# chrismile/LineVis

Hardware: AMD Instinct MI355X
Metric: Mrays/s (higher is better)
Workload: dtype f32

## Files before the change

### linevis_amd/csrc/lv_api.hip

```cpp
#include <algorithm>
#include <cmath>
#include <cstdlib>
#include <cstring>

#include "lv_internal.h"
#include "lv_trace.h"
#include "lv_mboit.h"

int lv_fail(lv_ctx* ctx, int code, const char* fmt, ...) {
    char buf[1024];
    va_list ap;
    va_start(ap, fmt);
    vsnprintf(buf, sizeof(buf), fmt, ap);
    va_end(ap);
    if (ctx) ctx->lastError = buf;
    return code;
}

int lv_buf_reserve(lv_ctx* ctx, LvDeviceBuffer& b, size_t bytes) {
    if (bytes == 0) bytes = 16;
    if (b.ptr && b.bytes >= bytes) return LV_OK;
    if (b.ptr) {
        LV_HIP(ctx, hipStreamSynchronize(ctx->stream));
        (void)hipFree(b.ptr);
// ... 33 lines not shown
    float c14 = m[4] * m[15] - m[12] * m[7];
    float c15 = m[4] * m[11] - m[8] * m[7];
    float c16 = m[8] * m[14] - m[12] * m[10];
    float c18 = m[4] * m[14] - m[12] * m[6];
    float c19 = m[4] * m[10] - m[8] * m[6];
    float c20 = m[8] * m[13] - m[12] * m[9];
    float c22 = m[4] * m[13] - m[12] * m[5];
    float c23 = m[4] * m[9] - m[8] * m[5];

    float i00 = +((m[5] * c00 - m[6] * c04) + m[7] * c08);
    float i01 = -((m[1] * c00 - m[2] * c04) + m[3] * c08);
    float i02 = +((m[1] * c02 - m[2] * c06) + m[3] * c10);
    float i03 = -((m[1] * c03 - m[2] * c07) + m[3] * c11);
    float i10 = -((m[4] * c00 - m[6] * c12) + m[7] * c16);
    float i11 = +((m[0] * c00 - m[2] * c12) + m[3] * c16);
    float i12 = -((m[0] * c02 - m[2] * c14) + m[3] * c18);
    float i13 = +((m[0] * c03 - m[2] * c15) + m[3] * c19);
    float i20 = +((m[4] * c04 - m[5] * c12) + m[7] * c20);
    float i21 = -((m[0] * c04 - m[1] * c12) + m[3] * c20);
    float i22 = +((m[0] * c06 - m[1] * c14) + m[3] * c22);
    float i23 = -((m[0] * c07 - m[1] * c15) + m[3] * c23);
    float i30 = -((m[4] * c08 - m[5] * c16) + m[6] * c20);
    float i31 = +((m[0] * c08 - m[1] * c16) + m[2] * c20);
    float i32 = -((m[0] * c10 - m[1] * c18) + m[2] * c22);
    float i33 = +((m[0] * c11 - m[1] * c19) + m[2] * c23);

    float det = ((m[0] * i00 + m[1] * i10) + m[2] * i20) + m[3] * i30;
    float r = 1.0f / det;
    inv[0] = i00 * r;  inv[1] = i01 * r;  inv[2] = i02 * r;  inv[3] = i03 * r;
    inv[4] = i10 * r;  inv[5] = i11 * r;  inv[6] = i12 * r;  inv[7] = i13 * r;
    inv[8] = i20 * r;  inv[9] = i21 * r;  inv[10] = i22 * r; inv[11] = i23 * r;
    inv[12] = i30 * r; inv[13] = i31 * r; inv[14] = i32 * r; inv[15] = i33 * r;
    return det;
}

static bool lv_mat4_invertible(const float* m, const float* inv, float det) {
    float hadamard = 1.0f;
    for (int c = 0; c < 4; c++) hadamard *= sqrtf(((m[4 * c] * m[4 * c] + m[4 * c + 1] * m[4 * c + 1]) + m[4 * c + 2] * m[4 * c + 2]) + m[4 * c + 3] * m[4 * c + 3]);
    for (int i = 0; i < 16; i++)
        if (!std::isfinite(m[i]) || !std::isfinite(inv[i])) return false;
    return std::isfinite(det) && std::isfinite(hadamard) && fabsf(det) > 1e-5f * hadamard;
}

static std::vector<LvDeviceBuffer*> lv_all_buffers(lv_ctx* ctx) {
    return {&ctx->points, &ctx->segIdx, &ctx->nodes, &ctx->segs, &ctx->segAxis, &ctx->prismFrames, &ctx->leafSeg, &ctx->segToLeaf, &ctx->tf,
            &ctx->depthMinMax, &ctx->ao, &ctx->aoAlt, &ctx->featNormal, &ctx->featNormalAlt, &ctx->featPosition, &ctx->featPositionAlt,
            &ctx->eawPing, &ctx->eawPong, &ctx->tilesHaloDev, &ctx->fullFrameTile, &ctx->svgf.normalDepth, &ctx->svgf.normalDepthHistory,
            &ctx->svgf.flowFwidth, &ctx->svgf.moments, &ctx->svgf.momentsHistory, &ctx->svgf.colorHistory, &ctx->svgf.tempAccum,
            &ctx->svgf.tempAccumFiltered, &ctx->svgf.ping, &ctx->svgf.pong, &ctx->svgf.result, &ctx->svgfGiven, &ctx->aoGbuf, &ctx->aoList, &ctx->aoSamples,
            &ctx->counters, &ctx->ppllNodes, &ctx->ppllStart, &ctx->ppllCount, &ctx->ppllScratch, &ctx->prismRecords, &ctx->scanTemp, &ctx->ppllOverflow, &ctx->mlabLong, &ctx->mlabStatsSnap, &ctx->mboitAccum, &ctx->ppllCoarse, &ctx->prismLeafList, &ctx->flowOccupancy, &ctx->flowPoints, &ctx->flowPointsNext, &ctx->flowSelfGrid, &ctx->twistTex, &ctx->tilesDev, &ctx->outDev,
            &ctx->scratchRays, &ctx->stackOverflow, &ctx->trajPos, &ctx->trajAttr, &ctx->trajOff, &ctx->trajLineValid, &ctx->trajLineRef, &ctx->trajRecLine, &ctx->trajTess, &ctx->trajRibbon, &ctx->trajHelicity, &ctx->trajMaxHelicity, &ctx->trajRecPoint, &ctx->trajMeshRot, &ctx->triIdx, &ctx->triVerts, &ctx->triPoints, &ctx->triNodes, &ctx->tris, &ctx->triPairFlag,
            &ctx->flowVectors, &ctx->flowScalars, &ctx->flowMisc, &ctx->flowSeeds, &ctx->flowOutPos, &ctx->flowOutAtt, &ctx->flowCounts,
            &ctx->bakeBlendingWeights, &ctx->bakeSamplingLocations, &ctx->bakedAo, &ctx->bakeLcgSkip, &ctx->bakedAoPending, &ctx->bakeCounters,
            &ctx->bakeGbuf, &ctx->bakeSamples, &ctx->bakeOverflow, &ctx->mlatTrace, &ctx->buildArena, &ctx->firstHit,
            &ctx->accum, &ctx->selftestIn, &ctx->selftestOut, &ctx->groupOrder[0].cost, &ctx->groupOrder[0].order, &ctx->groupOrder[1].cost, &ctx->groupOrder[1].order};
}

namespace {

typedef LvDevCounters LvDevCountersHost;

bool parseBool(const char* v) { return strcmp(v, "true") == 0 || strcmp(v, "1") == 0; }

bool parseFloat(const char* v, float& out) {
    char* end = nullptr;
    float f = strtof(v, &end);
    if (end == v) return false;
    out = f;
    return true;
}
bool parseUint(const char* v, uint32_t& out) {
    char* end = nullptr;
    long long x = strtoll(v, &end, 10);
    if (end == v || x < 0 || x > 0xFFFFFFFFll) return false;
    out = uint32_t(x);
    return true;
}

void updateAoMode(lv_ctx* ctx) {
    ctx->opt.useAmbientOcclusion = ctx->opt.aoBakerIsRtao && ctx->opt.aoStrength > 0.0f;
}

}

extern "C" {

const char* lv_version(void) { return "linevis_hip 0.1 (gfx950)"; }

lv_ctx* lv_create(int device_ordinal, int* err) {
    int n = 0;
    hipError_t e = hipGetDeviceCount(&n);
    if (e != hipSuccess || n <= 0 || device_ordinal < 0 || device_ordinal >= n) {
        if (err) *err = LV_E_HIP;
        return nullptr;
    }
    if (hipSetDevice(device_ordinal) != hipSuccess) {
        if (err) *err = LV_E_HIP;
        return nullptr;
    }
    lv_ctx* ctx = new lv_ctx();
    ctx->device = device_ordinal;
    {
        hipDeviceProp_t prop;
        if (hipGetDeviceProperties(&prop, device_ordinal) == hipSuccess && prop.multiProcessorCount > 0)
            ctx->numCUs = prop.multiProcessorCount;
    }
    memset(&ctx->stats, 0, sizeof(ctx->stats));
// ... 563 lines not shown
        if (p != o.triLeafPairs) { ctx->triAccelValid = false; lv_invalidate_bake(ctx); }
        o.triLeafPairs = p;
    } else if (k == "treelet_leaves") {
        uint32_t t;
        if (!parseUint(value, t) || t < 3 || t > 4096) return bad();
        if (t != o.treeletLeaves) { ctx->accelValid = false; ctx->triAccelValid = false; lv_invalidate_bake(ctx); }
        o.treeletLeaves = t;
    } else if (k == "treelet_lane_leaves") {
        uint32_t t;
        if (!parseUint(value, t) || t == 1 || t > 64) return bad();
        if (t != o.treeletLaneLeaves) { ctx->accelValid = false; ctx->triAccelValid = false; lv_invalidate_bake(ctx); }
        o.treeletLaneLeaves = t;
    } else if (k == "treelet_group_leaves") {
        uint32_t t;
        if (!parseUint(value, t) || (t != 0 && t != 8 && t != 16)) return bad();
        if (t != o.treeletGroupLeaves) { ctx->accelValid = false; ctx->triAccelValid = false; lv_invalidate_bake(ctx); }
        o.treeletGroupLeaves = t;
    } else if (k == "kernel_timers") {
        const std::string v(value);
        uint32_t mask = 0u;
        if (v == "all") mask = 0xFFFFFFFFu;
        else if (v != "none") {
            size_t pos = 0;
            while (pos <= v.size()) {
                size_t e = v.find(',', pos);
                if (e == std::string::npos) e = v.size();
                const std::string t = v.substr(pos, e - pos);
                pos = e + 1;
                uint32_t id;
                if (t == "phases") mask |= 1u << 31;
                else if (parseUint(t.c_str(), id) && id < 31u) mask |= 1u << id;
                else return bad();
            }
        }
        o.timerMask = mask;
    } else if (k == "accel_collapse_top") {
        const bool b = parseBool(value);
        if (b != o.collapseTop) { ctx->accelValid = false; ctx->triAccelValid = false; lv_invalidate_bake(ctx); }
        o.collapseTop = b;
    } else if (k == "treelet_plane_eval") {
        bool sc;
        if (std::string(value) == "scan") sc = true;
        else if (std::string(value) == "loop") sc = false;
        else return bad();
        if (sc != o.treeletPlaneScan) { ctx->accelValid = false; ctx->triAccelValid = false; lv_invalidate_bake(ctx); }
        o.treeletPlaneScan = sc;
    } else if (k == "accel_build") {
        bool ft;
        if (std::string(value) == "fast_trace") ft = true;
        else if (std::string(value) == "fast_build") ft = false;
        else return bad();
        if (ft != o.accelFastTrace) { ctx->accelValid = false; ctx->triAccelValid = false; lv_invalidate_bake(ctx); }
        o.accelFastTrace = ft;
    } else if (k == "dispatch_order") {
        if (std::string(value) == "cost") o.dispatchByCost = true;
        else if (std::string(value) == "as_numbered") o.dispatchByCost = false;
        else return bad();
    } else if (k == "rtao_geometry") {
        if (std::string(value) == "auto") o.rtaoGeometry = 0;
        else if (std::string(value) == "capsules") o.rtaoGeometry = 1;
        else if (std::string(value) == "triangle_tubes") o.rtaoGeometry = 2;
        else return bad();
    } else {
        return lv_fail(ctx, LV_E_INVALID, "unknown option '%s'", key);
    }
    return lv_forward_to_ranks(ctx, [&](lv_ctx* p) { return lv_set_option(p, key, value); });
}

int lv_build_accel(lv_ctx* ctx) {
    if (!ctx) return LV_E_INVALID;
    (void)hipSetDevice(ctx->device);
    int rc = lv_ensure_line_points(ctx);
    if (rc) return rc;
    if ((rc = lv_bvh_build(ctx))) return rc;
    const bool needTriangles = (ctx->opt.useAmbientOcclusion && (ctx->opt.aoPrebaked || lv_ao_triangle_tubes(ctx))) || ctx->opt.rtTriangleMesh;
    if (needTriangles) {
        if ((rc = lv_ensure_tube_mesh(ctx))) return rc;
        if (ctx->triMeshSet && (rc = lv_bvh_build_triangles(ctx))) return rc;
    }
    return lv_forward_to_ranks(ctx, [&](lv_ctx* p) { return lv_build_accel(p); });
}

lv_ctx* lv_create_multi(const int* device_ordinals, int num_devices, const char* transport, int* err) {
    if (!device_ordinals || num_devices <= 0) {
        if (err) *err = LV_E_INVALID;
        return nullptr;
    }
    lv_ctx* ctx = lv_create(device_ordinals[0], err);
    if (!ctx) return nullptr;
    const int rc = lv_multi_create(ctx, device_ordinals, num_devices, transport);
    if (rc) {
        fprintf(stderr, "lv_create_multi: %s\n", ctx->lastError.c_str());
        lv_destroy(ctx);
        if (err) *err = rc;
        return nullptr;
    }
    if (err) *err = LV_OK;
    return ctx;
}

int lv_multi_ranks(const lv_ctx* ctx) { return ctx ? lv_multi_num_ranks(ctx) : 0; }

int lv_multi_rebalance(lv_ctx* ctx, double base_cost_per_tile) {
    if (!ctx) return LV_E_INVALID;
    return lv_multi_rebalance_impl(ctx, base_cost_per_tile);
}
// ... 606 lines not shown
```

### linevis_amd/csrc/lv_bvh.hip

```cpp
#include <algorithm>
#include <cstring>
#include <utility>

#include <rocprim/device/device_radix_sort.hpp>
#include <rocprim/device/device_scan.hpp>

#include "lv_internal.h"

namespace {

__device__ __forceinline__ void lv_block_bounds(const float mn[3], const float mx[3], uint32_t* boundsOrd) {
    __shared__ float s_red[6][LV_BLOCK / LV_WAVE];
#pragma unroll
    for (int k = 0; k < 3; k++) {
        const float a = lv_wave_min(mn[k]), b = lv_wave_max(mx[k]);
        if (lv_lane() == 0) { s_red[k][threadIdx.x >> 6] = a; s_red[3 + k][threadIdx.x >> 6] = b; }
    }
    __syncthreads();
    if (threadIdx.x < 6) {
        float v = s_red[threadIdx.x][0];
        for (int w = 1; w < LV_BLOCK / LV_WAVE; w++)
            v = threadIdx.x < 3 ? fminf(v, s_red[threadIdx.x][w]) : fmaxf(v, s_red[threadIdx.x][w]);
        if (threadIdx.x < 3) atomicMin(&boundsOrd[threadIdx.x], lv_f2ord(v));
        else atomicMax(&boundsOrd[threadIdx.x], lv_f2ord(v));
// ... 774 lines not shown
                    const bool valid = j < hi;
                    bool left = false;
                    uint32_t e = 0;
                    if (valid) {
                        e = s_idx[j];
                        const float* b = s_box[e];
                        const int bi = int(((b[ax] + b[3 + ax]) - cmn[ax]) * scale[ax]);
                        const uint32_t bn = uint32_t(bi < 0 ? 0 : (bi > int(LV_TREELET_BINS) - 1 ? int(LV_TREELET_BINS) - 1 : bi));
                        left = bn < plane;
                    }
                    const unsigned long long mL = __ballot(left), mR = __ballot(valid && !left);
                    if (valid) {
                        if (left) s_tmp[lo + runL + uint32_t(__popcll(mL & below))] = e;
                        else s_tmp[lo + nl + runR + uint32_t(__popcll(mR & below))] = e;
                    }
                    runL += uint32_t(__popcll(mL));
                    runR += uint32_t(__popcll(mR));
                }
                LV_TREELET_SYNC();
                for (uint32_t j = lo + lane; j < hi; j += 64u) s_idx[j] = s_tmp[j];
                LV_TREELET_SYNC();
                if (nl == 0u || nl == n) nl = n / 2u;
            }
        }
        const uint32_t nr = n - nl;
        const uint32_t sL = nl > 1u ? v++ : 0u, sR = nr > 1u ? v++ : 0u;
        if (lane == 0u) {
            childL[slot] = nl > 1u ? sL : ((a + s_idx[lo]) | LV_LEAF_BIT);
            childR[slot] = nr > 1u ? sR : ((a + s_idx[lo + nl]) | LV_LEAF_BIT);
            if (nl == 2u) { childL[sL] = (a + s_idx[lo]) | LV_LEAF_BIT; childR[sL] = (a + s_idx[lo + 1u]) | LV_LEAF_BIT; }
            if (nr == 2u) { childL[sR] = (a + s_idx[lo + nl]) | LV_LEAF_BIT; childR[sR] = (a + s_idx[lo + nl + 1u]) | LV_LEAF_BIT; }
        }
        const bool goL = nl > 2u, goR = nr > 2u;
        if (goL && goR) {
            const bool leftFirst = nl <= nr;
            const uint32_t plo = leftFirst ? lo + nl : lo, phi = leftFirst ? hi : lo + nl, pslot = leftFirst ? sR : sL;
            const uint32_t nF = leftFirst ? nl : nr;
            if (lane == 0u) { s_stack[4 * sp] = plo; s_stack[4 * sp + 1] = phi; s_stack[4 * sp + 2] = pslot; s_stack[4 * sp + 3] = v + nF - 2u; }
            sp++;
            if (leftFirst) { hi = lo + nl; slot = sL; } else { lo = lo + nl; slot = sR; }
        } else if (goL) {
            hi = lo + nl; slot = sL;
        } else if (goR) {
            lo = lo + nl; slot = sR;
        } else {
            if (sp == 0u) break;
            sp--;
            LV_TREELET_SYNC();
            lo = s_stack[4 * sp]; hi = s_stack[4 * sp + 1]; slot = s_stack[4 * sp + 2]; v = s_stack[4 * sp + 3];
        }
        LV_TREELET_SYNC();
    }
    if (nSmall || nMid) runSmall();
}

__global__ __launch_bounds__(LV_BLOCK) void k_refit_pass(uint32_t nInternal, uint32_t pass, const uint32_t* __restrict__ childL,
                                                         const uint32_t* __restrict__ childR,
                                                         const float* __restrict__ leafBox, float* nodeBox,
                                                         uint32_t* height, uint32_t* done) {
    const uint32_t i = blockIdx.x * LV_BLOCK + threadIdx.x;
    if (i >= nInternal || done[i] != 0u) return;
    const uint32_t cl = childL[i], cr = childR[i];
    uint32_t hl = 0, hr = 0;
    const float *bl, *br;
    if (cl & LV_LEAF_BIT) bl = leafBox + 6 * size_t(cl & ~LV_LEAF_BIT);
    else {
        const uint32_t d = done[cl];
        if (d == 0u || d >= pass) return;
        bl = nodeBox + 6 * size_t(cl);
        hl = height[cl];
    }
    if (cr & LV_LEAF_BIT) br = leafBox + 6 * size_t(cr & ~LV_LEAF_BIT);
    else {
        const uint32_t d = done[cr];
        if (d == 0u || d >= pass) return;
        br = nodeBox + 6 * size_t(cr);
        hr = height[cr];
    }
#pragma unroll
    for (int k = 0; k < 3; k++) {
        nodeBox[6 * size_t(i) + k] = fminf(bl[k], br[k]);
        nodeBox[6 * size_t(i) + 3 + k] = fmaxf(bl[k + 3], br[k + 3]);
    }
    height[i] = max(hl, hr) + 1u;
    done[i] = pass;
}

__device__ __forceinline__ float lv_dec(float origin, float scale, uint32_t q) { return __builtin_fmaf(float(q), scale, origin); }

__device__ __forceinline__ void lv_write_wide_node(float4* out, int ns, const uint32_t slotRef[4], const float b[4][6]) {
    float origin[3], scale[3];
    uint32_t qmin[3] = {0, 0, 0}, qmax[3] = {0, 0, 0};
#pragma unroll
    for (int a = 0; a < 3; a++) {
        float lo = 3.0e38f, hi = -3.0e38f;
#pragma unroll
        for (int k = 0; k < 4; k++)
            if (k < ns) { lo = fminf(lo, b[k][a]); hi = fmaxf(hi, b[k][3 + a]); }
        origin[a] = lo;
        float sc = (hi - lo) / 255.0f;
        sc = sc * 1.000002f + 1e-30f;
        scale[a] = sc;
#pragma unroll
        for (int k = 0; k < 4; k++) {
            if (k >= ns) continue;
            int q0 = int(floorf((b[k][a] - lo) / sc));
// ... 189 lines not shown
            wideIndex, slots;
    auto freeAll = [&]() {};
#define LV_TRY(expr)                 \
    do {                             \
        int _rc = (expr);            \
        if (_rc) { freeAll(); return _rc; } \
    } while (0)
#define LV_HIPF(expr)                                                                                     \
    do {                                                                                                  \
        hipError_t _e = (expr);                                                                           \
        if (_e != hipSuccess) {                                                                           \
            freeAll();                                                                                    \
            return lv_fail(ctx, LV_E_HIP, "%s failed: %s (%s:%d)", #expr, hipGetErrorString(_e), __FILE__, __LINE__); \
        }                                                                                                 \
    } while (0)
    if (!ctx->pinned) LV_HIPF(hipHostMalloc((void**)&ctx->pinned, 64, hipHostMallocDefault));
    volatile uint32_t* pin = ctx->pinned;
    size_t sortBytes = 0, scanBytes = 0;
    LV_HIPF(rocprim::radix_sort_pairs(nullptr, sortBytes, (uint64_t*)nullptr, (uint64_t*)nullptr, (uint32_t*)nullptr,
                                      (uint32_t*)nullptr, n, 0, 63, st));
    LV_HIPF(rocprim::exclusive_scan(nullptr, scanBytes, (uint32_t*)nullptr, (uint32_t*)nullptr, 0u, nInternal,
                                    rocprim::plus<uint32_t>(), st));
    {
        struct Req { Tmp* t; size_t bytes; };
        const Req reqs[] = {{&boxOrig, size_t(n) * 24}, {&leafBox, size_t(n) * 24}, {&nodeBox, size_t(nInternal) * 24},
                            {&keysA, size_t(n) * 8}, {&keysB, size_t(n) * 8}, {&valsA, size_t(n) * 4}, {&valsB, size_t(n) * 4},
                            {&childL, size_t(nInternal) * 4}, {&childR, size_t(nInternal) * 4},
                            {&height, size_t(nInternal) * 4}, {&flags, size_t(nInternal) * 4}, {&bounds, 6 * 4},
                            {&sortTmp, std::max<size_t>(std::max(sortBytes, scanBytes), 16)},
                            {&depth, size_t(nInternal) * 4}, {&evenFlag, size_t(nInternal) * 4},
                            {&wideIndex, size_t(nInternal) * 4}, {&slots, size_t(nInternal) * 16}};
        size_t total = 0;
        for (const Req& r : reqs) total += (r.bytes + 255) & ~size_t(255);
        LV_TRY(lv_buf_reserve(ctx, ctx->buildArena, total));
        size_t off = 0;
        for (const Req& r : reqs) { r.t->ptr = (char*)ctx->buildArena.ptr + off; off += (r.bytes + 255) & ~size_t(255); }
    }

    if (timed) LV_HIPF(hipEventRecord(ctx->ev[evBase], st));
    {
        uint32_t* init = ctx->pinned + 8;
        init[0] = init[1] = init[2] = 0xFFFFFFFFu;
        init[3] = init[4] = init[5] = 0u;
        LV_HIPF(hipMemcpyAsync(bounds.ptr, init, 24, hipMemcpyHostToDevice, st));
    }
    boxes((float*)boxOrig.ptr, (uint32_t*)bounds.ptr);
    k_morton<<<nblocks(n), LV_BLOCK, 0, st>>>((const float*)boxOrig.ptr, n, (const uint32_t*)bounds.ptr,
                                              (uint64_t*)keysA.ptr, (uint32_t*)valsA.ptr);
    {
        size_t tmpBytes = sortBytes;
        LV_HIPF(rocprim::radix_sort_pairs(sortTmp.ptr, tmpBytes, (uint64_t*)keysA.ptr, (uint64_t*)keysB.ptr,
                                          (uint32_t*)valsA.ptr, (uint32_t*)valsB.ptr, n, 0, 63, st));
    }
    leaves((const uint32_t*)valsB.ptr, (const float*)boxOrig.ptr, (float*)leafBox.ptr);
    if (n == 1) {
        k_single_node<<<1, 64, 0, st>>>((const float*)leafBox.ptr, (float4*)nodesOut.ptr);
    } else {
        LV_HIPF(hipMemsetAsync(flags.ptr, 0, size_t(nInternal) * 4, st));
        k_karras<<<nblocks(nInternal), LV_BLOCK, 0, st>>>((const uint64_t*)keysB.ptr, int(n), (uint32_t*)childL.ptr,
                                                          (uint32_t*)childR.ptr, (uint32_t*)depth.ptr, (uint32_t*)evenFlag.ptr);
        if (ctx->opt.accelFastTrace && n >= 3u) {
            LV_HIPF(hipMemsetAsync(height.ptr, 0, 4, st));
            k_treelet_roots<<<nblocks(nInternal), LV_BLOCK, 0, st>>>(nInternal, (const uint32_t*)childL.ptr, (const uint32_t*)childR.ptr,
                                                                     (const uint32_t*)depth.ptr, (const uint32_t*)evenFlag.ptr,
                                                                     ctx->opt.treeletLeaves, (uint32_t*)wideIndex.ptr,
                                                                     (uint32_t*)height.ptr);
            LV_HIPF(hipMemcpyAsync((void*)ctx->pinned, height.ptr, 4, hipMemcpyDeviceToHost, st));
            LV_HIPF(hipStreamSynchronize(st));
            const uint32_t numTreelets = pin[0];
            if (numTreelets) {
                const size_t ldsBytes = size_t(ctx->opt.treeletLeaves) * 32;
                int maxLds = 0;
                LV_HIPF(hipDeviceGetAttribute(&maxLds, hipDeviceAttributeMaxSharedMemoryPerBlock, ctx->device));
                if (ldsBytes > size_t(maxLds)) {
                    freeAll();
                    return lv_fail(ctx, LV_E_INVALID, "treelet_leaves = %u needs %zu bytes of LDS per workgroup, the device has %d",
                                   ctx->opt.treeletLeaves, ldsBytes, maxLds);
                }
                auto* kernel = ctx->opt.treeletPlaneScan ? k_treelet_rebuild<true> : k_treelet_rebuild<false>;
                if (ldsBytes > 48 * 1024)
                    LV_HIPF(hipFuncSetAttribute((const void*)kernel, hipFuncAttributeMaxDynamicSharedMemorySize, int(ldsBytes)));
                kernel<<<numTreelets, 64, ldsBytes, st>>>(
                        (const uint32_t*)wideIndex.ptr, (const uint32_t*)depth.ptr, (const uint32_t*)evenFlag.ptr,
                        (const float*)leafBox.ptr, ctx->opt.treeletLeaves, ctx->opt.treeletLaneLeaves, ctx->opt.treeletGroupLeaves,
                        (uint32_t*)childL.ptr, (uint32_t*)childR.ptr);
            }
        }
        for (uint32_t pass = 1;; pass++) {
            k_refit_pass<<<nblocks(nInternal), LV_BLOCK, 0, st>>>(nInternal, pass, (const uint32_t*)childL.ptr,
                                                                  (const uint32_t*)childR.ptr, (const float*)leafBox.ptr,
                                                                  (float*)nodeBox.ptr, (uint32_t*)height.ptr,
                                                                  (uint32_t*)flags.ptr);
            if (pass % 8u == 0u) {
                LV_HIPF(hipMemcpyAsync((void*)ctx->pinned, flags.ptr, 4, hipMemcpyDeviceToHost, st));
                LV_HIPF(hipStreamSynchronize(st));
                if (pin[0]) break;
                if (pass > 4096u) { freeAll(); return lv_fail(ctx, LV_E_HIP, "LBVH refit did not converge"); }
            }
        }
        {
            uint32_t* frontier = (uint32_t*)depth.ptr;
            uint32_t* nextFrontier = (uint32_t*)evenFlag.ptr;
            uint32_t count = 1, base = 0;
            if (ctx->opt.collapseTop) {
                k_collapse_top<<<1, LV_BLOCK, 0, st>>>((const uint32_t*)childL.ptr, (const uint32_t*)childR.ptr, (const float*)leafBox.ptr,
                                                       (const float*)nodeBox.ptr, frontier, (float4*)nodesOut.ptr,
// ... 139 lines not shown
```

### linevis_amd/csrc/lv_internal.h

```cpp
#pragma once

#include <hip/hip_runtime.h>

#include <cstdarg>
#include <cstdio>
#include <map>
#include <string>
#include <vector>

#include "lv_device.h"

struct LvDeviceBuffer {
    void* ptr = nullptr;
    size_t bytes = 0;
};

struct LvSvgfState {
    LvDeviceBuffer normalDepth, normalDepthHistory;
    LvDeviceBuffer flowFwidth;
    LvDeviceBuffer moments, momentsHistory;
    LvDeviceBuffer colorHistory;
    LvDeviceBuffer tempAccum, tempAccumFiltered;
    LvDeviceBuffer ping, pong;
    LvDeviceBuffer result;
    uint32_t width = 0, height = 0;
    bool historyValid = false;
};

struct LvOptions {
    float lineWidth = 0.002f;
    float depthCueStrength = 0.0f;
    bool useAmbientOcclusion = false;
    bool aoBakerIsRtao = false;
    float aoStrength = 0.0f;
    float aoGamma = 1.0f;
    uint32_t aoIterations = 64;
    uint32_t aoSamplesPerFrame = 4;
    float aoRadius = 0.1f;
    bool aoUseDistance = true;
    uint32_t triLeafSize = 2;
    bool triLeafPairs = true;
    uint32_t treeletLeaves = 512;
    uint32_t treeletLaneLeaves = 6;
    uint32_t treeletGroupLeaves = 16;
    uint32_t timerMask = 0xFFFFFFFFu;
    bool collapseTop = true;
    bool treeletPlaneScan = true;
    bool accelFastTrace = true;
    bool fastShading = false;
    int overlapPrimaryPasses = 2;
    bool dispatchByCost = true;
    bool aoJitterPrimary = true;
    bool traceRaysHardwareInv = false;
    bool aoPixelGeneration = true;
    uint32_t numSamplesPerFrame = 1;
    uint32_t numAccumulatedFrames = 1;
    uint32_t frameNumber = 0;
    bool useDeterministicSampling = false;
    uint32_t maxDepthComplexity = 1024;
    bool useCappedTubes = true;
    bool useHalos = true;
    uint32_t tubeNumSubdivisions = 6;
    uint32_t ppllSortingMode = 0;
    uint32_t ppllMaxNumFrags = 0;
    uint32_t ppllExpectedAvgDepthComplexity = 0;
    uint32_t ppllTileW = 2, ppllTileH = 8;
    bool collectStats = false;
    bool aoPrebaked = false;
    uint32_t bakeIterations = 128;
    uint32_t bakeNumTubeSubdivisions = 8;
    uint32_t bakeSamplesPerFrame = 4;
    bool rtLss = false;
    bool rtTriangleMesh = false;
    int rtaoGeometry = 0;
    bool useMlat = false;
    uint32_t mlatNumNodes = 8;
    uint32_t mlabNumLayers = 8;
    uint32_t mboitNumMoments = 4;
    float mboitOverestimation = 0.1f;
    float mboitMomentBias = 0.0f;
    bool mboitStreamed = false;
    bool eawEnabled = false;
    uint32_t eawIterations = 3;
    bool eawColorWeights = true, eawPositionWeights = true, eawNormalWeights = true;
    float eawPhiColor = 0.49f, eawPhiPosition = 0.3f, eawPhiNormal = 0.1f;
    bool eawUseSharedMemory = true;
    bool useRibbons = false, thickBands = true, ellipticTubes = false;
    float bandWidth = 0.005f, minBandThickness = 0.15f;
    bool helicityBands = false, uniformTwistLineWidth = true;
    float separatorWidth = 0.2f, helicityRotationFactor = 1.0f;
    bool useTwistLineTexture = false;
    uint32_t twistFilterMode = 5;
    uint32_t bandSubdivisions = 6;
    bool svgfEnabled = false;
    uint32_t svgfIterations = 5;
    float svgfAllowedZDist = 0.002f, svgfAllowedNormalDist = 0.02f;
    int intersectionForm = 0;
    int ppllFragmentSource = 0;
    bool ppllPrismLbvhWalk = false;
    bool ppllRayTracerColour = false;
    bool mlatRecordTrace = false;
// ... 64 lines not shown
    float view[16] = {}, proj[16] = {}, invView[16] = {}, invProj[16] = {};
    float fovY = 0.0f, nearDist = 0.01f, farDist = 100.0f;
    uint32_t width = 0, height = 0;
    float background[4] = {1.0f, 1.0f, 1.0f, 1.0f};

    LvOptions opt;

    LvDeviceBuffer depthMinMax;
    LvDeviceBuffer ao;
    LvDeviceBuffer aoAlt;
    LvDeviceBuffer featNormal, featNormalAlt, featPosition, featPositionAlt;
    LvDeviceBuffer eawPing, eawPong;
    const float* aoResult = nullptr;
    bool aoRestart = false;
    LvSvgfState svgf;
    LvDeviceBuffer svgfGiven;
    LvDeviceBuffer fullFrameTile;
    uint32_t aoGlobalFrameNumber = 0;
    float lastFrameViewProj[16] = {};
    bool lastFrameViewProjValid = false;
    uint32_t tilesHalo = 0;
    LvDeviceBuffer tilesHaloDev;
    std::vector<uint32_t> tilesHaloHost;
    bool tilesHaloUploaded = false;
    uint32_t aoNumGroups = 0, aoGroupsPerTile = 0;
    LvDeviceBuffer aoGbuf, aoList, aoSamples;
    LvDeviceBuffer firstHit;
    LvDeviceBuffer counters;
    LvDeviceBuffer ppllNodes, ppllStart, ppllCount, ppllScratch;
    LvDeviceBuffer prismRecords, scanTemp;
    uint32_t ppllScanBlocks = 0;
    LvDeviceBuffer twistTex;
    uint32_t twistW = 0, twistH = 0, twistLevels = 0;
    LvDeviceBuffer flowOccupancy;
    LvDeviceBuffer flowPoints, flowPointsNext;
    size_t flowPointsCapacity = 0;
    LvDeviceBuffer flowSelfGrid;
    LvDeviceBuffer prismLeafList;
    LvDeviceBuffer ppllCoarse;
    LvDeviceBuffer ppllOverflow;
    LvDeviceBuffer mlabLong;
    LvDeviceBuffer mlabStatsSnap;
    uint64_t mlabPoolSlots = 0;
    uint32_t mboitBoxOrd[6] = {0, 0, 0, 0, 0, 0};
    bool mboitBoxValid = false;
    LvDeviceBuffer mboitAccum;
    bool mboitStreamLast = false, mboitStreamFull = false;
    uint32_t mboitStreamW = 0, mboitStreamH = 0, mboitStreamN = 0, mboitStreamTile[2] = {0, 0};
    bool ppllArrays = false;
    LvDeviceBuffer tilesDev, outDev, scratchRays, stackOverflow, mlatTrace;
    LvDeviceBuffer selftestIn, selftestOut;
    LvDeviceBuffer accum;
    uint32_t* pinned = nullptr;
    LvDeviceBuffer buildArena;
    struct GroupOrder {
        LvDeviceBuffer cost, order;
        uint32_t n = 0, tileW = 0, tileH = 0;
        uint64_t generation = ~0ull;
        bool active = false;
    } groupOrder[2];
    bool groupOrderSorted = false;
    uint64_t tilesGeneration = 0;
    bool tilesCoverViewport = false;
    uint32_t tilesCoverKey[4] = {0, 0, 0, 0};
    std::vector<uint32_t> tilesHost;
    bool tilesUploaded = false;
    uint64_t ppllPoolNodes = 0;
    uint32_t aoW = 0, aoH = 0, ppllPaddedW = 0, ppllPaddedH = 0, accumW = 0, accumH = 0;

    lv_stats stats;
    hipEvent_t ev[16];
    bool evCreated = false;
    bool evBuildValid = false, evFrameValid = false, evPhaseRecorded = false;
    bool evTriBuildValid = false;
    bool evLinePointsValid = false, evTessValid = false;
    int lastMode = 0;
    static constexpr int kNumKernels = 8;
    static constexpr int kRing = 512;
    hipEvent_t evKernel[kNumKernels][2 * kRing];
    uint64_t kernelLaunches[kNumKernels] = {0, 0, 0, 0, 0, 0, 0, 0};
};

int lv_fail(lv_ctx* ctx, int code, const char* fmt, ...);
inline bool lv_ao_triangle_tubes(const lv_ctx* ctx) {
    return ctx->opt.rtaoGeometry == 2 || (ctx->opt.rtaoGeometry == 0 && (ctx->triMeshSet || ctx->trajSet));
}
inline bool lv_literal_intersection(const lv_ctx* ctx) {
    if (ctx->opt.intersectionForm != 0) return ctx->opt.intersectionForm == 2;
    return !(ctx->opt.useAmbientOcclusion && !ctx->opt.aoPrebaked && !lv_ao_triangle_tubes(ctx));
}
inline float lv_accel_width(const lv_ctx* ctx) {
    return (ctx->opt.useRibbons && ctx->opt.ellipticTubes) ? ctx->opt.bandWidth : ctx->opt.lineWidth;
}

#define LV_HIP(ctx, expr)                                                                          \
    do {                                                                                           \
        hipError_t _e = (expr);                                                                    \
        if (_e != hipSuccess)                                                                      \
            return lv_fail(ctx, LV_E_HIP, "%s failed: %s (%s:%d)", #expr, hipGetErrorString(_e), __FILE__, __LINE__); \
    } while (0)

int lv_buf_reserve(lv_ctx* ctx, LvDeviceBuffer& b, size_t bytes);
inline hipEvent_t lv_kernel_ev(lv_ctx* ctx, int id, int which) {
    return ctx->evKernel[id][2 * (ctx->kernelLaunches[id] % lv_ctx::kRing) + which];
}
#define LV_TIMED_LAUNCH(ctx, id, launch)                                      \
// ... 76 lines not shown
```

Before: 5343.

## Add top-down binned SAH partitioning pass before Morton-based BVH build

Adds a GPU top-down partition that splits primitives into clusters, choosing each split by binned SAH cost using wave-aggregated shared-memory hash bins, down to treelet-sized clusters. Each primitive's split path is prepended to its Morton key and the primitives are re-sorted, so the upper tree levels follow SAH splits instead of Morton order. The goal is better tree quality for faster ray traversal, at the price of extra build time and a per-level host synchronisation. It is enabled by default for scenes of at least 65536 leaves when the fast-trace build mode is on.

```diff
diff --git a/linevis_amd/csrc/lv_api.hip b/linevis_amd/csrc/lv_api.hip
--- a/linevis_amd/csrc/lv_api.hip
+++ b/linevis_amd/csrc/lv_api.hip
@@ -109,7 +109,7 @@
             &ctx->scratchRays, &ctx->stackOverflow, &ctx->trajPos, &ctx->trajAttr, &ctx->trajOff, &ctx->trajLineValid, &ctx->trajLineRef, &ctx->trajRecLine, &ctx->trajTess, &ctx->trajRibbon, &ctx->trajHelicity, &ctx->trajMaxHelicity, &ctx->trajRecPoint, &ctx->trajMeshRot, &ctx->triIdx, &ctx->triVerts, &ctx->triPoints, &ctx->triNodes, &ctx->tris, &ctx->triPairFlag,
             &ctx->flowVectors, &ctx->flowScalars, &ctx->flowMisc, &ctx->flowSeeds, &ctx->flowOutPos, &ctx->flowOutAtt, &ctx->flowCounts,
             &ctx->bakeBlendingWeights, &ctx->bakeSamplingLocations, &ctx->bakedAo, &ctx->bakeLcgSkip, &ctx->bakedAoPending, &ctx->bakeCounters,
-            &ctx->bakeGbuf, &ctx->bakeSamples, &ctx->bakeOverflow, &ctx->mlatTrace, &ctx->buildArena, &ctx->firstHit,
+            &ctx->bakeGbuf, &ctx->bakeSamples, &ctx->bakeOverflow, &ctx->mlatTrace, &ctx->buildArena, &ctx->partitionScratch, &ctx->firstHit,
             &ctx->accum, &ctx->selftestIn, &ctx->selftestOut, &ctx->groupOrder[0].cost, &ctx->groupOrder[0].order, &ctx->groupOrder[1].cost, &ctx->groupOrder[1].order};
 }
 
@@ -779,6 +779,18 @@
         else return bad();
         if (ft != o.accelFastTrace) { ctx->accelValid = false; ctx->triAccelValid = false; lv_invalidate_bake(ctx); }
         o.accelFastTrace = ft;
+    } else if (k == "accel_partition") {
+        bool sah;
+        if (std::string(value) == "sah") sah = true;
+        else if (std::string(value) == "morton") sah = false;
+        else return bad();
+        if (sah != o.accelPartitionSah) { ctx->accelValid = false; ctx->triAccelValid = false; lv_invalidate_bake(ctx); }
+        o.accelPartitionSah = sah;
+    } else if (k == "accel_partition_min_leaves") {
+        uint32_t t;
+        if (!parseUint(value, t)) return bad();
+        if (t != o.accelPartitionMinLeaves) { ctx->accelValid = false; ctx->triAccelValid = false; lv_invalidate_bake(ctx); }
+        o.accelPartitionMinLeaves = t;
     } else if (k == "dispatch_order") {
         if (std::string(value) == "cost") o.dispatchByCost = true;
         else if (std::string(value) == "as_numbered") o.dispatchByCost = false;
diff --git a/linevis_amd/csrc/lv_bvh.hip b/linevis_amd/csrc/lv_bvh.hip
--- a/linevis_amd/csrc/lv_bvh.hip
+++ b/linevis_amd/csrc/lv_bvh.hip
@@ -850,6 +850,270 @@
         LV_TREELET_SYNC();
     }
     if (nSmall || nMid) runSmall();
+}
+
+#define LV_PART_LEVELS 32u
+#define LV_PART_MAX_CLUSTERS 65536u
+#define LV_PART_BIN_WORDS 13u
+#define LV_PART_WORD_IS_MIN(w) ((w) % LV_PART_BIN_WORDS < 3u || ((w) % LV_PART_BIN_WORDS >= 7u && (w) % LV_PART_BIN_WORDS < 10u))
+#define LV_PART_CLUSTER_WORDS (3u * LV_TREELET_BINS * LV_PART_BIN_WORDS)
+#define LV_PART_FINAL 0x80000000u
+
+__device__ __forceinline__ uint32_t lv_part_bin(float lo, float hi, float cmn, float scale) {
+    const int bi = int(((lo + hi) - cmn) * scale);
+    return uint32_t(bi < 0 ? 0 : (bi > int(LV_TREELET_BINS) - 1 ? int(LV_TREELET_BINS) - 1 : bi));
+}
+__device__ __forceinline__ void lv_part_axis(const float* cen, int ax, float& cmn, float& scale) {
+    cmn = cen[ax];
+    const float ext = cen[3 + ax] - cmn;
+    scale = ext > 0.0f ? float(LV_TREELET_BINS) / ext : 0.0f;
+}
+
+__global__ void k_part_init(uint32_t* __restrict__ bins, uint32_t* __restrict__ counters) {
+    const uint32_t t = threadIdx.x;
+    for (uint32_t w = t; w < LV_PART_CLUSTER_WORDS; w += blockDim.x) bins[w] = LV_PART_WORD_IS_MIN(w) ? 0xFFFFFFFFu : 0u;
+    if (t < LV_PART_LEVELS + 1u) counters[t] = t == 0u ? 1u : 0u;
+    if (t < 6u) counters[LV_PART_LEVELS + 1u + t] = t < 3u ? 0xFFFFFFFFu : 0u;
+}
+__global__ __launch_bounds__(LV_BLOCK) void k_part_root_centres(const float* __restrict__ boxOrig, uint32_t n, uint32_t* __restrict__ cenOrd) {
+    float mn[3] = {3.0e38f, 3.0e38f, 3.0e38f}, mx[3] = {-3.0e38f, -3.0e38f, -3.0e38f};
+    for (uint32_t s = blockIdx.x * LV_BLOCK + threadIdx.x; s < n; s += gridDim.x * LV_BLOCK)
+#pragma unroll
+        for (int k = 0; k < 3; k++) {
+            const float c = boxOrig[6 * size_t(s) + k] + boxOrig[6 * size_t(s) + 3 + k];
+            mn[k] = fminf(mn[k], c);
+            mx[k] = fmaxf(mx[k], c);
+        }
+    lv_block_bounds(mn, mx, cenOrd);
+}
+__global__ void k_part_root(const uint32_t* __restrict__ cenOrd, float* __restrict__ clusterCen) {
+    if (threadIdx.x < 6u) clusterCen[threadIdx.x] = lv_ord2f(cenOrd[threadIdx.x]);
+}
+
+#define LV_PART_ITEMS 8u
+#define LV_PART_SLOTS 512u
+#define LV_PART_PROBES 4u
+__device__ __forceinline__ void lv_part_add(uint32_t* w, const float mn[3], const float mx[3], const float cmn[3], const float cmx[3], uint32_t count) {
+#pragma unroll
+    for (int k = 0; k < 3; k++) {
+        atomicMin(&w[k], lv_f2ord(mn[k]));
+        atomicMax(&w[3 + k], lv_f2ord(mx[k]));
+        atomicMin(&w[7 + k], lv_f2ord(cmn[k]));
+        atomicMax(&w[10 + k], lv_f2ord(cmx[k]));
+    }
+    atomicAdd(&w[6], count);
+}
+template <bool BIN>
+__global__ __launch_bounds__(LV_BLOCK) void k_part_level(const float* __restrict__ boxOrig, const uint32_t* __restrict__ order, uint32_t n, uint32_t first, uint32_t maxClusters,
+                                                         uint32_t* __restrict__ state, uint32_t* __restrict__ path,
+                                                         const uint32_t* __restrict__ splitPrev, const float* __restrict__ boxPrev,
+                                                         const float* __restrict__ boxCur, uint32_t* __restrict__ bins) {
+    __shared__ uint32_t s_tag[BIN ? LV_PART_SLOTS : 1u];
+    __shared__ uint32_t s_val[BIN ? LV_PART_SLOTS : 1u][LV_PART_BIN_WORDS];
+    if (BIN) {
+        for (uint32_t j = threadIdx.x; j < LV_PART_SLOTS; j += LV_BLOCK) {
+            s_tag[j] = LV_INVALID;
+#pragma unroll
+            for (uint32_t w = 0; w < LV_PART_BIN_WORDS; w++) s_val[j][w] = LV_PART_WORD_IS_MIN(w) ? 0xFFFFFFFFu : 0u;
+        }
+        __syncthreads();
+    }
+#pragma unroll 1
+    for (uint32_t it = 0; it < LV_PART_ITEMS; it++) {
+        const uint32_t s = (blockIdx.x * LV_PART_ITEMS + it) * LV_BLOCK + threadIdx.x;
+        bool active = s < n;
+        uint32_t st = 0u;
+        float b[6] = {0.0f, 0.0f, 0.0f, 0.0f, 0.0f, 0.0f};
+        if (active) {
+            st = first ? 0u : state[s];
+            active = !(st & LV_PART_FINAL);
+        }
+        if (active) {
+#pragma unroll
+            for (int k = 0; k < 6; k++) b[k] = boxOrig[6 * size_t(order[s]) + k];
+            if (!first) {
+                const uint32_t c = st & 0xFFFFu, len = (st >> 16) & 0xFFu;
+                const uint32_t sp = splitPrev[3u * c];
+                if (sp == LV_INVALID) {
+                    st |= LV_PART_FINAL;
+                } else {
+                    const int ax = int(sp & 3u);
+                    float cmn, scale;
+                    lv_part_axis(boxPrev + 6 * size_t(c), ax, cmn, scale);
+                    const uint32_t side = lv_part_bin(b[ax], b[3 + ax], cmn, scale) >= (sp >> 2) ? 1u : 0u;
+                    const uint32_t child = splitPrev[3u * c + 1u + side];
+                    path[s] = (len ? path[s] << 1 : 0u) | side;
+                    st = (child < maxClusters ? child : LV_PART_FINAL) | ((len + 1u) << 16);
+                }
+                state[s] = st;
+                active = !(st & LV_PART_FINAL);
+            } else {
+                state[s] = 0u;
+                path[s] = 0u;
+            }
+        }
+        if (!BIN) continue;
+        const uint32_t c = st & 0xFFFFu;
+        uint32_t key[3] = {LV_INVALID, LV_INVALID, LV_INVALID};
+        if (active) {
+#pragma unroll
+            for (int ax = 0; ax < 3; ax++) {
+                float cmn, scale;
+                lv_part_axis(boxCur + 6 * size_t(c), ax, cmn, scale);
+                key[ax] = (c * 3u + uint32_t(ax)) * LV_TREELET_BINS + lv_part_bin(b[ax], b[3 + ax], cmn, scale);
+            }
+        }
+        auto merge = [&](bool mine, uint32_t lk, int leader, int numKeys, const uint32_t* lks) {
+            const unsigned long long m = __ballot(mine);
+            float mn[3], mx[3], cmn[3], cmx[3];
+#pragma unroll
+            for (int k = 0; k < 3; k++) {
+                mn[k] = lv_wave_min(mine ? b[k] : 3.0e38f);
+                mx[k] = lv_wave_max(mine ? b[3 + k] : -3.0e38f);
+                cmn[k] = lv_wave_min(mine ? b[k] + b[3 + k] : 3.0e38f);
+                cmx[k] = lv_wave_max(mine ? b[k] + b[3 + k] : -3.0e38f);
+            }
+            if (int(lv_lane()) == leader) {
+                for (int q = 0; q < numKeys; q++) {
+                    const uint32_t kq = numKeys == 1 ? lk : lks[q];
+                    uint32_t slot = (kq * 2654435761u) >> 23;
+                    uint32_t* w = nullptr;
+                    for (uint32_t p = 0; p < LV_PART_PROBES && !w; p++, slot = (slot + 1u) & (LV_PART_SLOTS - 1u)) {
+                        const uint32_t prev = atomicCAS(&s_tag[slot], LV_INVALID, kq);
+                        if (prev == LV_INVALID || prev == kq) w = s_val[slot];
+                    }
+                    if (!w) w = bins + size_t(kq) * LV_PART_BIN_WORDS;
+                    lv_part_add(w, mn, mx, cmn, cmx, uint32_t(__popcll(m)));
+                }
+            }
+            return m;
+        };
+        const unsigned long long act = __ballot(active);
+        if (act == 0ull) continue;
+        const int first0 = __ffsll((long long)act) - 1;
+        const uint32_t lks[3] = {uint32_t(__shfl(int(key[0]), first0, 64)), uint32_t(__shfl(int(key[1]), first0, 64)),
+                                 uint32_t(__shfl(int(key[2]), first0, 64))};
+        if (__ballot(active && (key[0] != lks[0] || key[1] != lks[1] || key[2] != lks[2])) == 0ull) {
+            merge(active, 0u, first0, 3, lks);
+            continue;
+        }
+#pragma unroll 1
+        for (int ax = 0; ax < 3; ax++) {
+            const uint32_t kx = ax == 0 ? key[0] : (ax == 1 ? key[1] : key[2]);
+            unsigned long long todo = act;
+            while (todo) {
+                const int leader = __ffsll((long long)todo) - 1;
+                const uint32_t lk = uint32_t(__shfl(int(kx), leader, 64));
+                todo &= ~merge(active && kx == lk, lk, leader, 1, lks);
+            }
+        }
+    }
+    if (!BIN) return;
+    __syncthreads();
+    for (uint32_t j = threadIdx.x; j < LV_PART_SLOTS; j += LV_BLOCK) {
+        const uint32_t lk = s_tag[j];
+        if (lk == LV_INVALID) continue;
+        uint32_t* w = bins + size_t(lk) * LV_PART_BIN_WORDS;
+#pragma unroll
+        for (int k = 0; k < 3; k++) {
+            atomicMin(&w[k], s_val[j][k]);
+            atomicMax(&w[3 + k], s_val[j][3 + k]);
+            atomicMin(&w[7 + k], s_val[j][7 + k]);
+            atomicMax(&w[10 + k], s_val[j][10 + k]);
+        }
+        atomicAdd(&w[6], s_val[j][6]);
+    }
+}
+
+__global__ __launch_bounds__(64) void k_part_pick(uint32_t level, uint32_t maxLeaves, uint32_t maxClusters, const uint32_t* __restrict__ bins,
+                                                  uint32_t* __restrict__ split, float* __restrict__ boxNext, uint32_t* __restrict__ binsNext,
+                                                  uint32_t* __restrict__ counters) {
+    __shared__ uint32_t s_bin[3u * LV_TREELET_BINS][LV_PART_BIN_WORDS];
+    __shared__ uint32_t s_child[2];
+    const uint32_t lane = threadIdx.x;
+    const uint32_t count = min(counters[level], maxClusters);
+    for (uint32_t c = blockIdx.x; c < count; c += gridDim.x) {
+        __syncthreads();
+        if (lane < 3u * LV_TREELET_BINS)
+            for (uint32_t k = 0; k < LV_PART_BIN_WORDS; k++) s_bin[lane][k] = bins[(size_t(c) * 3u * LV_TREELET_BINS + lane) * LV_PART_BIN_WORDS + k];
+        if (lane < 2u) s_child[lane] = LV_INVALID;
+        __syncthreads();
+        float mn[2][3], mx[2][3], cmn[2][3], cmx[2][3];
+        uint32_t cn[2] = {0u, 0u};
+#pragma unroll
+        for (int h = 0; h < 2; h++)
+#pragma unroll
+            for (int k = 0; k < 3; k++) { mn[h][k] = cmn[h][k] = 3.0e38f; mx[h][k] = cmx[h][k] = -3.0e38f; }
+        unsigned long long key = ~0ull;
+        const uint32_t ax = lane / (LV_TREELET_BINS - 1u), plane = lane % (LV_TREELET_BINS - 1u) + 1u;
+        if (lane < 3u * (LV_TREELET_BINS - 1u)) {
+            for (uint32_t bn = 0; bn < LV_TREELET_BINS; bn++) {
+                const uint32_t* w = s_bin[ax * LV_TREELET_BINS + bn];
+                if (w[6] == 0u) continue;
+                const int h = bn < plane ? 0 : 1;
+                cn[h] += w[6];
+#pragma unroll
+                for (int k = 0; k < 3; k++) {
+                    mn[h][k] = fminf(mn[h][k], lv_ord2f(w[k]));
+                    mx[h][k] = fmaxf(mx[h][k], lv_ord2f(w[3 + k]));
+                    cmn[h][k] = fminf(cmn[h][k], lv_ord2f(w[7 + k]));
+                    cmx[h][k] = fmaxf(cmx[h][k], lv_ord2f(w[10 + k]));
+                }
+            }
+            if (cn[0] != 0u && cn[1] != 0u) {
+                float area[2];
+#pragma unroll
+                for (int h = 0; h < 2; h++) {
+                    const float dx = mx[h][0] - mn[h][0], dy = mx[h][1] - mn[h][1], dz = mx[h][2] - mn[h][2];
+                    area[h] = dx * dy + dy * dz + dz * dx;
+                }
+                const float cost = area[0] * float(cn[0]) + area[1] * float(cn[1]);
+                if (cost >= 0.0f && cost < 3.0e38f) key = ((unsigned long long)__float_as_uint(cost) << 32) | lane;
+            }
+        }
+        unsigned long long best = key;
+#pragma unroll
+        for (int o = 32; o > 0; o >>= 1) {
+            const unsigned long long ok = (unsigned long long)__shfl_xor((long long)best, o, 64);
+            best = ok < best ? ok : best;
+        }
+        if (best == ~0ull) {
+            if (lane == 0u) split[3u * c] = LV_INVALID;
+            continue;
+        }
+        if (key == best) {
+            split[3u * c] = ax | (plane << 2);
+            for (int h = 0; h < 2; h++) {
+                uint32_t id = LV_INVALID;
+                if (cn[h] > maxLeaves) {
+                    id = atomicAdd(&counters[level + 1u], 1u);
+                    if (id < maxClusters) {
+#pragma unroll
+                        for (int k = 0; k < 3; k++) { boxNext[6 * size_t(id) + k] = cmn[h][k]; boxNext[6 * size_t(id) + 3 + k] = cmx[h][k]; }
+                    } else {
+                        id = LV_INVALID;
+                    }
+                }
+                split[3u * c + 1u + h] = id;
+                s_child[h] = id;
+            }
+        }
+        __syncthreads();
+        for (int h = 0; h < 2; h++) {
+            const uint32_t id = s_child[h];
+            if (id == LV_INVALID) continue;
+            for (uint32_t w = lane; w < LV_PART_CLUSTER_WORDS; w += 64u)
+                binsNext[size_t(id) * LV_PART_CLUSTER_WORDS + w] = LV_PART_WORD_IS_MIN(w) ? 0xFFFFFFFFu : 0u;
+        }
+    }
+}
+
+__global__ __launch_bounds__(LV_BLOCK) void k_part_keys(uint32_t n, const uint32_t* __restrict__ state, const uint32_t* __restrict__ path,
+                                                        uint64_t* __restrict__ keys) {
+    const uint32_t s = blockIdx.x * LV_BLOCK + threadIdx.x;
+    if (s >= n) return;
+    const uint32_t len = (state[s] >> 16) & 0xFFu;
+    if (len) keys[s] = (uint64_t(path[s]) << (63u - len)) | (keys[s] >> len);
 }
 
 __global__ __launch_bounds__(LV_BLOCK) void k_refit_pass(uint32_t nInternal, uint32_t pass, const uint32_t* __restrict__ childL,
@@ -1145,6 +1409,44 @@
         LV_HIPF(rocprim::radix_sort_pairs(sortTmp.ptr, tmpBytes, (uint64_t*)keysA.ptr, (uint64_t*)keysB.ptr,
                                           (uint32_t*)valsA.ptr, (uint32_t*)valsB.ptr, n, 0, 63, st));
     }
+    if (ctx->opt.accelFastTrace && ctx->opt.accelPartitionSah && n > ctx->opt.treeletLeaves && n >= ctx->opt.accelPartitionMinLeaves) {
+        const uint32_t maxLeaves = ctx->opt.treeletLeaves;
+        const uint32_t cap = std::min<uint32_t>(n / (maxLeaves + 1u) + 1u, LV_PART_MAX_CLUSTERS);
+        auto al = [](size_t b) { return (b + 255) & ~size_t(255); };
+        const size_t oPath = al(size_t(n) * 4), oCount = oPath + al(size_t(n) * 4), oSplit = oCount + 256,
+                     oBox = oSplit + al(size_t(cap) * 12), oBins = oBox + 2 * al(size_t(cap) * 24),
+                     binBytes = al(size_t(cap) * LV_PART_CLUSTER_WORDS * 4);
+        LV_TRY(lv_buf_reserve(ctx, ctx->partitionScratch, oBins + 2 * binBytes));
+        char* base = (char*)ctx->partitionScratch.ptr;
+        uint32_t *state = (uint32_t*)base, *path = (uint32_t*)(base + oPath), *counters = (uint32_t*)(base + oCount),
+                 *split = (uint32_t*)(base + oSplit);
+        float* cbox[2] = {(float*)(base + oBox), (float*)(base + oBox + al(size_t(cap) * 24))};
+        uint32_t* bins[2] = {(uint32_t*)(base + oBins), (uint32_t*)(base + oBins + binBytes)};
+        k_part_init<<<1, LV_BLOCK, 0, st>>>(bins[0], counters);
+        k_part_root_centres<<<std::min(nblocks(n), 2048u), LV_BLOCK, 0, st>>>((const float*)boxOrig.ptr, n, counters + LV_PART_LEVELS + 1u);
+        k_part_root<<<1, 64, 0, st>>>(counters + LV_PART_LEVELS + 1u, cbox[0]);
+        const uint32_t partBlocks = uint32_t((uint64_t(n) + LV_PART_ITEMS * LV_BLOCK - 1) / (LV_PART_ITEMS * LV_BLOCK));
+        uint32_t level = 0, count = 1;
+        while (true) {
+            const uint32_t cur = level & 1u;
+            k_part_level<true><<<partBlocks, LV_BLOCK, 0, st>>>((const float*)boxOrig.ptr, (const uint32_t*)valsB.ptr, n, level == 0u ? 1u : 0u, cap, state, path, split,
+                                                                cbox[cur ^ 1u], cbox[cur], bins[cur]);
+            k_part_pick<<<std::min(count, 4096u), 64, 0, st>>>(level, maxLeaves, cap, bins[cur], split, cbox[cur ^ 1u], bins[cur ^ 1u], counters);
+            LV_HIPF(hipMemcpyAsync((void*)ctx->pinned, counters + level + 1u, 4, hipMemcpyDeviceToHost, st));
+            LV_HIPF(hipStreamSynchronize(st));
+            count = pin[0];
+            level++;
+            if (count == 0u || count > cap || level == LV_PART_LEVELS) break;
+        }
+        k_part_level<false><<<partBlocks, LV_BLOCK, 0, st>>>((const float*)boxOrig.ptr, (const uint32_t*)valsB.ptr, n, 0u, cap, state, path, split,
+                                                             cbox[(level & 1u) ^ 1u], cbox[level & 1u], bins[level & 1u]);
+        k_part_keys<<<nblocks(n), LV_BLOCK, 0, st>>>(n, state, path, (uint64_t*)keysB.ptr);
+        size_t tmpBytes = sortBytes;
+        LV_HIPF(rocprim::radix_sort_pairs(sortTmp.ptr, tmpBytes, (uint64_t*)keysB.ptr, (uint64_t*)keysA.ptr,
+                                          (uint32_t*)valsB.ptr, (uint32_t*)valsA.ptr, n, 0, 63, st));
+        std::swap(keysA.ptr, keysB.ptr);
+        std::swap(valsA.ptr, valsB.ptr);
+    }
     leaves((const uint32_t*)valsB.ptr, (const float*)boxOrig.ptr, (float*)leafBox.ptr);
     if (n == 1) {
         k_single_node<<<1, 64, 0, st>>>((const float*)leafBox.ptr, (float4*)nodesOut.ptr);
diff --git a/linevis_amd/csrc/lv_internal.h b/linevis_amd/csrc/lv_internal.h
--- a/linevis_amd/csrc/lv_internal.h
+++ b/linevis_amd/csrc/lv_internal.h
@@ -47,6 +47,8 @@
     bool collapseTop = true;
     bool treeletPlaneScan = true;
     bool accelFastTrace = true;
+    bool accelPartitionSah = true;
+    uint32_t accelPartitionMinLeaves = 65536;
     bool fastShading = false;
     int overlapPrimaryPasses = 2;
     bool dispatchByCost = true;
@@ -217,6 +219,7 @@
     LvDeviceBuffer selftestIn, selftestOut;
     LvDeviceBuffer accum;
     uint32_t* pinned = nullptr;
+    LvDeviceBuffer partitionScratch;
     LvDeviceBuffer buildArena;
     struct GroupOrder {
         LvDeviceBuffer cost, order;
```

Result: faster. 5433, median of 6 (+1.7%).
